# 0xPolygonZero/plonky2

Measured on AMD Instinct MI355X. Metric: LDE+Poseidon-commit GFE/s, higher is better.
Workload: dtype u64 (Goldilocks)

## Files before the change

### plonky2_amd/csrc/gl_mul3.hpp

```cpp
#pragma once
#include "asm_block.h"
#include "gl.hpp"

namespace gl {

#define P2_SA "v[70:71]", "v70", "v71", "v[72:73]", "v72", "v73", "v[74:75]", "v74", "v75", "s[40:41]", "s[42:43]"
#define P2_SB "v[76:77]", "v76", "v77", "v[78:79]", "v78", "v79", "v[80:81]", "v80", "v81", "s[44:45]", "s[46:47]"
#define P2_SC "v[82:83]", "v82", "v83", "v[84:85]", "v84", "v85", "v[86:87]", "v86", "v87", "s[48:49]", "s[50:51]"

#define P2_ST1(P, P0, P1, M, M0, M1, Q, Q0, Q1, C1, C2, a0, a1, b0, b1, r0, r1) "v_mad_u64_u32 " P ", " C1 ", %[" a0 "], %[" b0 "], 0\n\t"
#define P2_ST2(P, P0, P1, M, M0, M1, Q, Q0, Q1, C1, C2, a0, a1, b0, b1, r0, r1) "v_mad_u64_u32 " M ", " C1 ", %[" a1 "], %[" b0 "], 0\n\t"
#define P2_ST3(P, P0, P1, M, M0, M1, Q, Q0, Q1, C1, C2, a0, a1, b0, b1, r0, r1) "v_mad_u64_u32 " M ", " C2 ", %[" a0 "], %[" b1 "], " M "\n\t"
#define P2_ST4(P, P0, P1, M, M0, M1, Q, Q0, Q1, C1, C2, a0, a1, b0, b1, r0, r1) "v_mad_u64_u32 " Q ", " C1 ", %[" a1 "], %[" b1 "], 0\n\t"
#define P2_ST5(P, P0, P1, M, M0, M1, Q, Q0, Q1, C1, C2, a0, a1, b0, b1, r0, r1) "v_add_co_u32 " P1 ", " C1 ", " P1 ", " M0 "\n\t"
#define P2_ST6(P, P0, P1, M, M0, M1, Q, Q0, Q1, C1, C2, a0, a1, b0, b1, r0, r1) "v_addc_co_u32 " Q0 ", " C1 ", " Q0 ", " M1 ", " C1 "\n\t"
#define P2_ST7(P, P0, P1, M, M0, M1, Q, Q0, Q1, C1, C2, a0, a1, b0, b1, r0, r1) "v_addc_co_u32 " Q1 ", " C1 ", " Q1 ", 0, " C1 "\n\t"
#define P2_ST8(P, P0, P1, M, M0, M1, Q, Q0, Q1, C1, C2, a0, a1, b0, b1, r0, r1) "v_subb_co_u32 " P0 ", " C1 ", " P0 ", " Q1 ", " C2 "\n\t"
#define P2_ST9(P, P0, P1, M, M0, M1, Q, Q0, Q1, C1, C2, a0, a1, b0, b1, r0, r1) "v_subb_co_u32 " P1 ", " C1 ", " P1 ", 0, " C1 "\n\t"
#define P2_ST10(P, P0, P1, M, M0, M1, Q, Q0, Q1, C1, C2, a0, a1, b0, b1, r0, r1) "v_mad_u64_u32 " P ", " C2 ", " Q0 ", -1, " P "\n\t"
#define P2_ST11(P, P0, P1, M, M0, M1, Q, Q0, Q1, C1, C2, a0, a1, b0, b1, r0, r1) "v_cndmask_b32 " M0 ", 0, 1, " C2 "\n\t"
#define P2_ST12(P, P0, P1, M, M0, M1, Q, Q0, Q1, C1, C2, a0, a1, b0, b1, r0, r1) "v_subb_co_u32 " M0 ", " C1 ", " M0 ", 0, " C1 "\n\t"
#define P2_ST13(P, P0, P1, M, M0, M1, Q, Q0, Q1, C1, C2, a0, a1, b0, b1, r0, r1) "v_add_u32 " P1 ", " P1 ", " M0 "\n\t"
#define P2_ST14(P, P0, P1, M, M0, M1, Q, Q0, Q1, C1, C2, a0, a1, b0, b1, r0, r1) "v_mad_i64_i32 %[" r0 "], " C1 ", " M0 ", -1, " P "\n\t"

// ... 207 lines not shown
    return ra;
#endif
}

#define P2_FD1(P, P0, P1, M, M0, M1, Q, Q0, Q1, C1, C2, a0, a1, b0, b1, r0, r1) "v_mad_u64_u32 " P ", " C1 ", %[" b1 "], -1, %[" a0 "]\n\t"
#define P2_FD2(P, P0, P1, M, M0, M1, Q, Q0, Q1, C1, C2, a0, a1, b0, b1, r0, r1) "v_add_co_u32 " P1 ", " C1 ", " P1 ", %[" b0 "]\n\t"
#define P2_FD3(P, P0, P1, M, M0, M1, Q, Q0, Q1, C1, C2, a0, a1, b0, b1, r0, r1) "v_cndmask_b32 " M0 ", 0, -1, " C1 "\n\t"
#define P2_FD4(P, P0, P1, M, M0, M1, Q, Q0, Q1, C1, C2, a0, a1, b0, b1, r0, r1) "v_mad_u64_u32 %[" r0 "], " C1 ", " M0 ", 1, " P "\n\t"

__host__ __device__ __forceinline__ u64 fold_row_c(u64 al, u64 ah) {
    u32 k1;
    u32 w1 = addc32((u32)(al >> 32), (u32)ah, 0u, &k1);
    u32 w2 = (u32)(ah >> 32) + k1;
    u64 lo64 = ((u64)w1 << 32) | (u32)al;
    u64 t = (u64)w2 * 0xFFFFFFFFu + lo64;
    return fold_carry(t, t < lo64);
}

__device__ __forceinline__ void fold3(const u64 al[3], const u64 ah[3], u64 y[3]) {
    if (!P2_ASM_INTERPRETED()) {
        for (int k = 0; k < 3; ++k) y[k] = fold_row_c(al[k], ah[k]);
        return;
    }
    u64 ra, rb, rc;
    P2_ASM(P2_ROW(P2_FD1) P2_ROW(P2_FD2) P2_ROW(P2_FD3) P2_ROW(P2_FD4),
           (P2_O([ra0], "=&v", ra), P2_O([rb0], "=&v", rb), P2_O([rc0], "=&v", rc)),
           (P2_I([xa0], "v", al[0]), P2_I([ya0], "v", (u32)ah[0]), P2_I([ya1], "v", (u32)(ah[0] >> 32)),
            P2_I([xb0], "v", al[1]), P2_I([yb0], "v", (u32)ah[1]), P2_I([yb1], "v", (u32)(ah[1] >> 32)),
            P2_I([xc0], "v", al[2]), P2_I([yc0], "v", (u32)ah[2]), P2_I([yc1], "v", (u32)(ah[2] >> 32))),
           ("v70", "v71", "v72", "v76", "v77", "v78", "v82", "v83", "v84", "s40", "s41", "s44", "s45", "s48", "s49"));
    y[0] = ra;
    y[1] = rb;
    y[2] = rc;
}
__device__ __forceinline__ u64 fold1(u64 al, u64 ah) {
    if (!P2_ASM_INTERPRETED()) return fold_row_c(al, ah);
    u64 ra;
    P2_ASM(P2_A1(P2_FD1, P2_SA) P2_A1(P2_FD2, P2_SA) P2_NOP P2_A1(P2_FD3, P2_SA) P2_A1(P2_FD4, P2_SA),
           (P2_O([ra0], "=&v", ra)), (P2_I([xa0], "v", al), P2_I([ya0], "v", (u32)ah), P2_I([ya1], "v", (u32)(ah >> 32))),
           ("v70", "v71", "v72", "s40", "s41"));
    return ra;
}

#define P2_FW1(P, P0, P1, M, M0, M1, Q, Q0, Q1, C1, C2, a0, a1, b0, b1, r0, r1) "v_mad_u64_u32 " P ", " C1 ", %[" b1 "], -1, %[" a0 "]\n\t"
#define P2_FW2(P, P0, P1, M, M0, M1, Q, Q0, Q1, C1, C2, a0, a1, b0, b1, r0, r1) "v_cndmask_b32 " M0 ", 0, -1, " C1 "\n\t"
#define P2_FW3(P, P0, P1, M, M0, M1, Q, Q0, Q1, C1, C2, a0, a1, b0, b1, r0, r1) "v_mad_u64_u32 " P ", " C1 ", " M0 ", 1, " P "\n\t"
#define P2_FW4 P2_FD2
#define P2_FW5 P2_FD3
#define P2_FW6 P2_FD4

__host__ __device__ __forceinline__ u64 fold_row_wide_c(u64 al, u64 ah) {
    u64 t = (ah >> 32) * 0xFFFFFFFFull + al;
    t += t < al ? 0xFFFFFFFFull : 0;
    const u64 u = t + (ah << 32);
    return u + (u < t ? 0xFFFFFFFFull : 0);
}

__device__ __forceinline__ void fold3w(const u64 al[3], const u64 ah[3], u64 y[3]) {
    if (!P2_ASM_INTERPRETED()) {
        for (int k = 0; k < 3; ++k) y[k] = fold_row_wide_c(al[k], ah[k]);
        return;
    }
    u64 ra, rb, rc;
    P2_ASM(P2_ROW(P2_FW1) P2_ROW(P2_FW2) P2_ROW(P2_FW3) P2_ROW(P2_FW4) P2_ROW(P2_FW5) P2_ROW(P2_FW6),
           (P2_O([ra0], "=&v", ra), P2_O([rb0], "=&v", rb), P2_O([rc0], "=&v", rc)),
           (P2_I([xa0], "v", al[0]), P2_I([ya0], "v", (u32)ah[0]), P2_I([ya1], "v", (u32)(ah[0] >> 32)),
            P2_I([xb0], "v", al[1]), P2_I([yb0], "v", (u32)ah[1]), P2_I([yb1], "v", (u32)(ah[1] >> 32)),
            P2_I([xc0], "v", al[2]), P2_I([yc0], "v", (u32)ah[2]), P2_I([yc1], "v", (u32)(ah[2] >> 32))),
           ("v70", "v71", "v72", "v76", "v77", "v78", "v82", "v83", "v84", "s40", "s41", "s44", "s45", "s48", "s49"));
    y[0] = ra;
    y[1] = rb;
    y[2] = rc;
}
__device__ __forceinline__ u64 fold1w(u64 al, u64 ah) {
    if (!P2_ASM_INTERPRETED()) return fold_row_wide_c(al, ah);
    u64 ra;
    P2_ASM(P2_A1(P2_FW1, P2_SA) P2_NOP P2_A1(P2_FW2, P2_SA) P2_A1(P2_FW3, P2_SA) P2_A1(P2_FW4, P2_SA) P2_NOP P2_A1(P2_FW5, P2_SA)
               P2_A1(P2_FW6, P2_SA),
           (P2_O([ra0], "=&v", ra)), (P2_I([xa0], "v", al), P2_I([ya0], "v", (u32)ah), P2_I([ya1], "v", (u32)(ah >> 32))),
           ("v70", "v71", "v72", "s40", "s41"));
    return ra;
}

}
```

### plonky2_amd/csrc/merkle.hpp

```cpp
#pragma once
#include "poseidon.hpp"
#include "poseidon4.hpp"
#include "poseidon16.hpp"
#include "ntt.hpp"

namespace merkle {
using gl::u32;
using gl::u64;

struct ColMajorReader {
    const u64 *m;
    size_t stride;
    __device__ __forceinline__ u64 operator()(size_t L, unsigned e) const { return m[(size_t)e * stride + L]; }
};
struct RowMajorReader {
    const u64 *m;
    size_t W;
    __device__ __forceinline__ u64 operator()(size_t L, unsigned e) const { return m[L * W + e]; }
};
struct FriPlanarReader {
    const u64 *p0, *p1;
    unsigned arity_bits;
    __device__ __forceinline__ u64 operator()(size_t L, unsigned e) const {
        const u64 *p = (e & 1) ? p1 : p0;
        return p[(L << arity_bits) + (e >> 1)];
    }
};

struct DigestPrefixedReader {
    const u64 *prefix;
    const u64 *m;
    size_t stride;
    __device__ __forceinline__ u64 operator()(size_t L, unsigned e) const {
        return e < 4 ? prefix[4 * L + e] : m[(size_t)(e - 4) * stride + L];
    }
};

__device__ __forceinline__ u64 *node_slot(u64 *digests, u64 *cap, unsigned h, unsigned level, size_t j) {
    if (level == h) return cap + 4 * j;
    size_t s = j >> (h - level);
    size_t jl = j & (((size_t)1 << (h - level)) - 1);
    size_t sub_digests = 2 * (((size_t)1 << h) - 1);
    size_t idx = 2 * (((jl >> 1) << (level + 1)) + ((size_t)1 << level) - 1) + (jl & 1);
    return digests + 4 * (s * sub_digests + idx);
}

template <class Reader>
__global__ void __launch_bounds__(256) hash_leaves_kernel(Reader rd, unsigned W, size_t leaf_offset, size_t leaf_count,
                                                         unsigned h, u64 *digests, u64 *cap) {
    size_t t = (size_t)blockIdx.x * blockDim.x + threadIdx.x;
    if (t >= leaf_count) return;
    const size_t L = leaf_offset + t;
    u64 s[12];
#pragma unroll
    for (int i = 0; i < 12; ++i) s[i] = 0;
    if (W <= 4) {
        for (unsigned i = 0; i < W; ++i) s[i] = rd(L, i);
    } else {
        for (unsigned off = 0; off < W; off += 8) {
            unsigned cnt = W - off < 8 ? W - off : 8;
#pragma unroll
            for (unsigned i = 0; i < 8; ++i)
                if (i < cnt) s[i] = rd(L, off + i);
            const unsigned next = off + 8 < W ? (W - off - 8 < 8 ? W - off - 8 : 8) : 0;
            const unsigned keep = off + 8 < W ? (next == 8 ? 0x8u : (0xFu << (next / 3)) & 0xFu) : 0x1u;
            poseidon::permute(s, keep, off + 8 < W ? (next == 8 ? 8 : -1) : 3);
        }
    }
    u64 *dst = node_slot(digests, cap, h, 0, L);
#pragma unroll
    for (int i = 0; i < 4; ++i) dst[i] = gl::canon(s[i]);
}

template <class Reader>
__global__ void __launch_bounds__(256) hash_leaves_chunks_kernel(Reader rd, unsigned W, size_t leaf_offset, size_t leaf_count,
                                                                unsigned h, u64 *digests, u64 *cap, unsigned off_begin,
                                                                unsigned off_end, u64 *state, size_t state_stride) {
    size_t t = (size_t)blockIdx.x * blockDim.x + threadIdx.x;
    if (t >= leaf_count) return;
    const size_t L = leaf_offset + t;
    u64 s[12];
#pragma unroll
    for (int i = 0; i < 12; ++i) s[i] = 0;
    if (off_begin) {
        const unsigned nxt = W - off_begin < 8 ? W - off_begin : 8;
#pragma unroll
        for (unsigned i = 0; i < 12; ++i)
            if (i >= 3 * (nxt / 3)) s[i] = state[(size_t)i * state_stride + t];
    }
    for (unsigned off = off_begin; off < off_end; off += 8) {
        unsigned cnt = W - off < 8 ? W - off : 8;
#pragma unroll
        for (unsigned i = 0; i < 8; ++i)
            if (i < cnt) s[i] = rd(L, off + i);
        const unsigned next = off + 8 < W ? (W - off - 8 < 8 ? W - off - 8 : 8) : 0;
        const unsigned keep = off + 8 < W ? (next == 8 ? 0x8u : (0xFu << (next / 3)) & 0xFu) : 0x1u;
        poseidon::permute(s, keep, off + 8 < W ? (next == 8 ? 8 : -1) : 3);
    }
    if (off_end >= W) {
        u64 *dst = node_slot(digests, cap, h, 0, L);
#pragma unroll
        for (int i = 0; i < 4; ++i) dst[i] = gl::canon(s[i]);
    } else {
        const unsigned nxt = W - off_end < 8 ? W - off_end : 8;
#pragma unroll
        for (unsigned i = 0; i < 12; ++i)
            if (i >= 3 * (nxt / 3)) state[(size_t)i * state_stride + t] = s[i];
    }
}

__global__ void __launch_bounds__(256) merkle_level_kernel(u64 *digests, u64 *cap, unsigned h, unsigned level,
                                                          size_t n_nodes) {
    size_t j = (size_t)blockIdx.x * blockDim.x + threadIdx.x;
    if (j >= n_nodes) return;
    const u64 *ch = node_slot(digests, cap, h, level - 1, 2 * j);
    u64 out[4];
    poseidon::two_to_one(ch, ch + 4, out);
    u64 *dst = node_slot(digests, cap, h, level, j);
#pragma unroll
    for (int i = 0; i < 4; ++i) dst[i] = out[i];
}

template <class Reader>
__global__ void __launch_bounds__(256) hash_leaves_quad_kernel(Reader rd, unsigned W, size_t leaf_offset, size_t leaf_count,
                                                              unsigned h, u64 *digests, u64 *cap) {
    const size_t t = ((size_t)blockIdx.x * blockDim.x + threadIdx.x) >> 2;
    const unsigned q = threadIdx.x & 3;
    const bool live = t < leaf_count;
    const size_t L = leaf_offset + (live ? t : 0);
    u64 w[3] = {0, 0, 0};
    if (W <= 4) {
#pragma unroll
        for (unsigned u = 0; u < 3; ++u)
            if (live && 3 * q + u < W) w[u] = rd(L, 3 * q + u);
    } else {
        for (unsigned off = 0; off < W; off += 8) {
            const unsigned cnt = W - off < 8 ? W - off : 8;
#pragma unroll
            for (unsigned u = 0; u < 3; ++u) {
                const unsigned e = 3 * q + u;
                if (live && e < cnt) w[u] = rd(L, off + e);
            }
            poseidon4::permute_quad(w, q);
        }
    }
    if (live) {
        u64 *dst = node_slot(digests, cap, h, 0, L);
        if (q == 0) {
            dst[0] = gl::canon(w[0]);
            dst[1] = gl::canon(w[1]);
            dst[2] = gl::canon(w[2]);
        } else if (q == 1) {
            dst[3] = gl::canon(w[0]);
        }
    }
}

__global__ void __launch_bounds__(256) merkle_level_quad_kernel(u64 *digests, u64 *cap, unsigned h, unsigned level,
                                                               size_t n_nodes) {
    const size_t j = ((size_t)blockIdx.x * blockDim.x + threadIdx.x) >> 2;
    const unsigned q = threadIdx.x & 3;
    const bool live = j < n_nodes;
    const u64 *ch = node_slot(digests, cap, h, level - 1, 2 * (live ? j : 0));
    u64 w[3];
#pragma unroll
    for (unsigned u = 0; u < 3; ++u) w[u] = (live && 3 * q + u < 8) ? ch[3 * q + u] : 0;
    poseidon4::permute_quad(w, q);
    if (live) {
        u64 *dst = node_slot(digests, cap, h, level, j);
        if (q == 0) {
            dst[0] = gl::canon(w[0]);
            dst[1] = gl::canon(w[1]);
            dst[2] = gl::canon(w[2]);
        } else if (q == 1) {
            dst[3] = gl::canon(w[0]);
        }
    }
}

template <class Reader>
// ... 38 lines not shown
    if (live) states[12 * t + r] = gl::canon(w);
}

__global__ void permute_batch_kernel(u64 *states, size_t count) {
    size_t t = (size_t)blockIdx.x * blockDim.x + threadIdx.x;
    if (t >= count) return;
    u64 s[12];
#pragma unroll
    for (int i = 0; i < 12; ++i) s[i] = states[12 * t + i];
    poseidon::permute(s);
#pragma unroll
    for (int i = 0; i < 12; ++i) states[12 * t + i] = gl::canon(s[i]);
}

__global__ void field_selftest_kernel(const u64 *a, const u64 *b, size_t count, u64 *out) {
    size_t t = (size_t)blockIdx.x * blockDim.x + threadIdx.x;
    if (t >= count) return;
    const u64 x = a[t], y = b[t];
    out[t] = gl::canon(gl::mul(x, y));
    out[count + t] = gl::canon(gl::mul1(x, y));
    u64 aa[3] = {x, y, x}, bb[3] = {y, x, x}, rr[3];
    gl::mul3(aa, bb, rr);
    u64 ok = (gl::canon(rr[1]) == gl::canon(rr[0])) && (gl::canon(rr[2]) == gl::canon(gl::mul(x, x))) ? 0 : 1;
    if (gl::canon(gl::mul1_lowregs(x, y)) != gl::canon(gl::mul(x, y))) ok |= 2;
#define P2_CHK_POW2(S)                                                                                              \
    if (gl::canon(ntt::mul_pow2_asm<S>(x)) != gl::canon(gl::mul(x, (S) < 64 ? 1ull << ((S) & 63) : 0xFFFFFFFFull << (((S) - 64) & 31)))) \
        ok |= 4;
    P2_CHK_POW2(12) P2_CHK_POW2(24) P2_CHK_POW2(36) P2_CHK_POW2(48) P2_CHK_POW2(60) P2_CHK_POW2(72) P2_CHK_POW2(84)
    P2_CHK_POW2(1) P2_CHK_POW2(31) P2_CHK_POW2(33) P2_CHK_POW2(63) P2_CHK_POW2(65) P2_CHK_POW2(95)
#undef P2_CHK_POW2
    {
        const u64 al = x >> 1, ah = y >> 1;
        const u64 want = gl::canon(gl::add(al, gl::mul(ah, 1ull << 32)));
        if (gl::canon(gl::fold1(al, ah)) != want) ok |= 8;
        const u64 al3[3] = {al, ah, al ^ 0x2AAAAAAAAAAAAAAAull}, ah3[3] = {ah, al, ah};
        u64 y3[3];
        gl::fold3(al3, ah3, y3);
        for (int k = 0; k < 3; ++k)
            if (gl::canon(y3[k]) != gl::canon(gl::add(al3[k], gl::mul(ah3[k], 1ull << 32)))) ok |= 16;
    }
    {
        const u64 a2[2] = {x, y ^ 0x9E3779B97F4A7C15ull}, b2[2] = {y, x};
        u64 r2[2];
        gl::mul2(a2, b2, r2);
        if (gl::canon(r2[0]) != gl::canon(gl::mul(x, y)) || gl::canon(r2[1]) != gl::canon(gl::mul(a2[1], x))) ok |= 32;
    }
    if (gl::canon(gl::mul_add(x, y, x ^ y)) != gl::canon(gl::add(gl::mul(x, y), x ^ y)) || gl::canon(gl::mul_add(y, x, ~0ull)) != gl::canon(gl::add(gl::mul(x, y), ~0ull)) ||
        gl::canon(gl::mul_add(x, x, y)) != gl::canon(gl::add(gl::mul(x, x), y)))
        ok |= 128;
    {
        const u64 a3[3] = {x, y, x}, b3[3] = {y, x, x}, c3[3] = {x ^ y, ~0ull, y};
        u64 r3[3];
        gl::mad3(a3, b3, c3, r3);
        for (int k = 0; k < 3; ++k)
            if (gl::canon(r3[k]) != gl::canon(gl::add(gl::mul(a3[k], b3[k]), c3[k]))) ok |= 256;
    }
    {
        const u64 a3[3] = {x, y, x ^ 0x9E3779B97F4A7C15ull}, b3[3] = {y, y, x};
        u64 r3[3];
        gl::mul3cg(a3, b3, r3);
        for (int k = 0; k < 3; ++k)
            if (gl::canon(r3[k]) != gl::canon(gl::mul(a3[k], b3[k]))) ok |= 512;
        if (gl::canon(gl::mul1cg(x, y)) != gl::canon(gl::mul(x, y)) || gl::canon(gl::mul1cg(y, y)) != gl::canon(gl::mul(y, y))) ok |= 512;
    }
    {
        const u64 al3[3] = {x, y, x ^ y}, ah3[3] = {y, x, ~x};
        u64 y3[3];
        gl::fold3w(al3, ah3, y3);
        for (int k = 0; k < 3; ++k)
            if (gl::canon(y3[k]) != gl::canon(gl::add(al3[k], gl::mul(ah3[k], 1ull << 32)))) ok |= 1024;
        if (gl::canon(gl::fold1w(x, y)) != gl::canon(gl::add(x, gl::mul(y, 1ull << 32)))) ok |= 1024;
    }
    {
        const u64 z = x ^ 0x9E3779B97F4A7C15ull;
        const u64 a3[3][3] = {{x, y, z}, {y, z, x}, {z, x, y}}, b3[3][3] = {{y, y, x}, {y, x, y}, {x, y, y}};
        for (int j = 0; j < 3; ++j) {
            u64 r3[3];
            gl::mul3cx(a3[j], b3[j], r3);
            for (int k = 0; k < 3; ++k)
                if (gl::canon(r3[k]) != gl::canon(gl::mul(a3[j][k], b3[j][k]))) ok |= 2048;
        }
        if (gl::canon(gl::mul1cx(x, y)) != gl::canon(gl::mul(x, y)) || gl::canon(gl::mul1cx(y, y)) != gl::canon(gl::mul(y, y))) ok |= 2048;
    }
    out[2 * count + t] = gl::canon(rr[0]);
    out[5 * count + t] = ok;
    out[3 * count + t] = gl::canon(gl::add(x, y));
    out[4 * count + t] = gl::canon(gl::sub(x, y));
}

}
```

### plonky2_amd/csrc/poseidon.hpp

```cpp
#pragma once
#include "gl.hpp"
#include "gl_mul3.hpp"
#ifndef P2HOT_EMU
#define P2_CONST_QUAL __constant__
#endif
#define P2_LITERAL_QUAL static constexpr
#include "poseidon_constants.h"

namespace poseidon {
using gl::u32;
using gl::u64;

#define RC P2_POSEIDON_ALL_ROUND_CONSTANTS
#define RC_SPLIT P2_POSEIDON_PUSHED_ROUND_CONSTANTS_SPLIT

__device__ __forceinline__ u64 sbox7(u64 x) {
    u64 x2 = gl::sqr(x);
    u64 x4 = gl::sqr(x2);
    u64 x3 = gl::mul(x, x2);
    return gl::mul(x3, x4);
}

__device__ __forceinline__ u64 ark(u64 a, u64 c) {
    if (!P2_ASM_INTERPRETED()) return gl::add_canon(a, c);
// ... 46 lines not shown
    b = x[1];
    c = x[2];
}

__device__ __forceinline__ void sbox_layer(u64 s[12]) {
#pragma unroll
    for (int i = 0; i < 12; i += 3) sbox7_x3(s[i], s[i + 1], s[i + 2]);
}
__device__ __forceinline__ void sbox_layer_cx(u64 s[12]) {
#pragma unroll
    for (int i = 0; i < 12; i += 3) sbox7_x3cx(s[i], s[i + 1], s[i + 2]);
}

__device__ __forceinline__ u32 opaque_const(u32 c) {
#ifndef P2HOT_EMU
    asm volatile("" : "+s"(c));
#endif
    return c;
}

template <u32 C>
__device__ __forceinline__ void mds_term(u64 (&al)[3], u64 (&ah)[3], u32 l0, u32 h0, u32 l1, u32 h1, u32 l2, u32 h2) {
    if (!P2_ASM_INTERPRETED()) {
        al[0] += (u64)l0 * C;
        ah[0] += (u64)h0 * C;
        al[1] += (u64)l1 * C;
        ah[1] += (u64)h1 * C;
        al[2] += (u64)l2 * C;
        ah[2] += (u64)h2 * C;
        return;
    }
    u64 d;
    P2_ASM_NC("v_mad_u64_u32 %0, %6, %7, %13, %0\n\t"
              "v_mad_u64_u32 %1, %6, %8, %13, %1\n\t"
              "v_mad_u64_u32 %2, %6, %9, %13, %2\n\t"
              "v_mad_u64_u32 %3, %6, %10, %13, %3\n\t"
              "v_mad_u64_u32 %4, %6, %11, %13, %4\n\t"
              "v_mad_u64_u32 %5, %6, %12, %13, %5",
              (P2_O(, "+v", al[0]), P2_O(, "+v", ah[0]), P2_O(, "+v", al[1]), P2_O(, "+v", ah[1]), P2_O(, "+v", al[2]),
               P2_O(, "+v", ah[2]), P2_O(, "=&s", d)),
              (P2_I(, "v", l0), P2_I(, "v", h0), P2_I(, "v", l1), P2_I(, "v", h1), P2_I(, "v", l2), P2_I(, "v", h2),
               P2_I(, "n", C)));
}
template <bool HAS_K>
__device__ __forceinline__ void mds_first(u64 (&al)[3], u64 (&ah)[3], u32 l0, u32 h0, u32 l1, u32 h1, u32 l2, u32 h2,
                                          const u64 *k) {
    if (!P2_ASM_INTERPRETED()) {
        const u64 z[6] = {0, 0, 0, 0, 0, 0};
        const u64 *kk = HAS_K ? k : z;
        al[0] = (u64)l0 * 17u + kk[0];
        ah[0] = (u64)h0 * 17u + kk[1];
        al[1] = (u64)l1 * 17u + kk[2];
        ah[1] = (u64)h1 * 17u + kk[3];
        al[2] = (u64)l2 * 17u + kk[4];
        ah[2] = (u64)h2 * 17u + kk[5];
        return;
    }
    u64 d;
    if (HAS_K) {
        P2_ASM_NC("v_mad_u64_u32 %0, %6, %7, 17, %13\n\t"
                  "v_mad_u64_u32 %1, %6, %8, 17, %14\n\t"
                  "v_mad_u64_u32 %2, %6, %9, 17, %15\n\t"
                  "v_mad_u64_u32 %3, %6, %10, 17, %16\n\t"
                  "v_mad_u64_u32 %4, %6, %11, 17, %17\n\t"
                  "v_mad_u64_u32 %5, %6, %12, 17, %18",
                  (P2_O(, "=&v", al[0]), P2_O(, "=&v", ah[0]), P2_O(, "=&v", al[1]), P2_O(, "=&v", ah[1]),
                   P2_O(, "=&v", al[2]), P2_O(, "=&v", ah[2]), P2_O(, "=&s", d)),
                  (P2_I(, "v", l0), P2_I(, "v", h0), P2_I(, "v", l1), P2_I(, "v", h1), P2_I(, "v", l2), P2_I(, "v", h2),
                   P2_I(, "s", k[0]), P2_I(, "s", k[1]), P2_I(, "s", k[2]), P2_I(, "s", k[3]), P2_I(, "s", k[4]),
                   P2_I(, "s", k[5])));
    } else {
        P2_ASM_NC("v_mad_u64_u32 %0, %6, %7, 17, 0\n\t"
                  "v_mad_u64_u32 %1, %6, %8, 17, 0\n\t"
                  "v_mad_u64_u32 %2, %6, %9, 17, 0\n\t"
                  "v_mad_u64_u32 %3, %6, %10, 17, 0\n\t"
                  "v_mad_u64_u32 %4, %6, %11, 17, 0\n\t"
                  "v_mad_u64_u32 %5, %6, %12, 17, 0",
                  (P2_O(, "=&v", al[0]), P2_O(, "=&v", ah[0]), P2_O(, "=&v", al[1]), P2_O(, "=&v", ah[1]),
                   P2_O(, "=&v", al[2]), P2_O(, "=&v", ah[2]), P2_O(, "=&s", d)),
                  (P2_I(, "v", l0), P2_I(, "v", h0), P2_I(, "v", l1), P2_I(, "v", h1), P2_I(, "v", l2), P2_I(, "v", h2)));
    }
}

template <int R>
__device__ __forceinline__ u64 mds_row(const u32 (&xl)[12], const u32 (&xh)[12]) {
    static_assert(R > 0 && R < 12, "row 0 carries the diagonal term");
    constexpr u32 C[12] = {17, 15, 41, 16, 2, 28, 13, 13, 39, 18, 34, 20};
    u64 al = (u64)xl[R] * opaque_const(C[0]), ah = (u64)xh[R] * opaque_const(C[0]);
#pragma unroll
    for (int i = 1; i < 12; ++i) {
        al += (u64)xl[(R + i) % 12] * opaque_const(C[i]);
        ah += (u64)xh[(R + i) % 12] * opaque_const(C[i]);
    }
    return gl::fold1(al, ah);
}

__device__ __forceinline__ void mds_layer(u64 s[12], const u64 *rc2, unsigned groups = 0xFu, int single = -1) {
    u32 xl[12], xh[12];
#pragma unroll
    for (int i = 0; i < 12; ++i) {
        xl[i] = (u32)s[i];
        xh[i] = (u32)(s[i] >> 32);
    }
#pragma unroll
    for (int g = 0; g < 12; g += 3) {
        if (!(groups >> (g / 3) & 1u)) continue;
        u64 al[3], ah[3], y[3];
#define P2_X(i) xl[(g + (i)) % 12], xh[(g + (i)) % 12], xl[(g + (i) + 1) % 12], xh[(g + (i) + 1) % 12], xl[(g + (i) + 2) % 12], xh[(g + (i) + 2) % 12]
        if (rc2)
            mds_first<true>(al, ah, P2_X(0), rc2 + 2 * g);
        else
            mds_first<false>(al, ah, P2_X(0), nullptr);
        mds_term<15>(al, ah, P2_X(1));
        mds_term<41>(al, ah, P2_X(2));
        mds_term<16>(al, ah, P2_X(3));
        mds_term<2>(al, ah, P2_X(4));
        mds_term<28>(al, ah, P2_X(5));
        mds_term<13>(al, ah, P2_X(6));
        mds_term<13>(al, ah, P2_X(7));
        mds_term<39>(al, ah, P2_X(8));
        mds_term<18>(al, ah, P2_X(9));
        mds_term<34>(al, ah, P2_X(10));
        mds_term<20>(al, ah, P2_X(11));
#undef P2_X
        if (g == 0) {
            al[0] += (u64)xl[0] * opaque_const(8);
            ah[0] += (u64)xh[0] * opaque_const(8);
        }
        gl::fold3(al, ah, y);
        s[g] = y[0];
        s[g + 1] = y[1];
        s[g + 2] = y[2];
    }
    if (single == 3)
        s[3] = mds_row<3>(xl, xh);
    else if (single == 8)
        s[8] = mds_row<8>(xl, xh);
}

struct Mat12 {
    u32 v[144];
};
constexpr Mat12 mds_matrix() {
    Mat12 m{};
    for (int r = 0; r < 12; ++r)
        for (int c = 0; c < 12; ++c) m.v[12 * r + c] = P2_POSEIDON_M1_ROW0[(c - r + 12) % 12] - ((c - r + 12) % 12 == 0 ? 8u : 0u) + (r == 0 && c == 0 ? 8u : 0u);
    return m;
}
constexpr Mat12 mat_mul(const Mat12 &a, const Mat12 &b) {
    Mat12 m{};
    for (int r = 0; r < 12; ++r)
        for (int c = 0; c < 12; ++c) {
            u64 acc = 0;
            for (int k = 0; k < 12; ++k) acc += (u64)a.v[12 * r + k] * b.v[12 * k + c];
            m.v[12 * r + c] = (u32)acc;
        }
    return m;
}
constexpr bool mat_checks() {
    const Mat12 m1 = mds_matrix(), m2 = mat_mul(m1, m1), m3 = mat_mul(m1, m2);
    for (int j = 0; j < 12; ++j) {
        if (m1.v[j] != P2_POSEIDON_M1_ROW0[j] || m2.v[j] != P2_POSEIDON_M2_ROW0[j]) return false;
        if (m1.v[12 * j] != P2_POSEIDON_MCOL0[j] || m2.v[12 * j] != P2_POSEIDON_MCOL0[12 + j]) return false;
    }
    for (int i = 0; i < 144; ++i)
        if (m3.v[i] != P2_POSEIDON_M3[i]) return false;
    return true;
}
static_assert(mat_checks(), "M, M^2, M^3: the compile-time products disagree with the generated tables");
constexpr Mat12 mat_drop_col0(const Mat12 &a) {
    Mat12 m = a;
    for (int r = 0; r < 12; ++r) m.v[12 * r] = 0;
    return m;
}
P2_LITERAL_QUAL Mat12 MDS1 = mds_matrix();
P2_LITERAL_QUAL Mat12 MDM = mat_mul(mat_drop_col0(mds_matrix()), mds_matrix());
P2_LITERAL_QUAL Mat12 MDMDM = mat_mul(mat_drop_col0(mds_matrix()), mat_mul(mat_drop_col0(mds_matrix()), mds_matrix()));
P2_LITERAL_QUAL Mat12 MDMDMDM = mat_mul(mat_drop_col0(mds_matrix()), MDMDM);

constexpr bool pass4_rows_fit() {
    const Mat12 m1 = mds_matrix(), md = mat_drop_col0(m1);
    const Mat12 p1 = mat_mul(md, m1), p2 = mat_mul(md, p1), p3 = mat_mul(md, p2);
    for (int i = 0; i < 144; ++i)
        if (p1.v[i] != MDM.v[i] || p2.v[i] != MDMDM.v[i] || p3.v[i] != MDMDMDM.v[i]) return false;
    for (int r = 0; r < 12; ++r) {
        u64 sum = (u64)p2.v[12 * r] + p1.v[12 * r] + m1.v[12 * r];
        for (int c = 0; c < 12; ++c) {
            u64 e = 0;
            for (int k = 0; k < 12; ++k) e += (u64)md.v[12 * r + k] * p2.v[12 * k + c];
            if (e != p3.v[12 * r + c]) return false;
            sum += e;
        }
        if (sum > (1ull << 32)) return false;
    }
    return true;
}
static_assert(pass4_rows_fit(), "(MD)^3 M: a four-application row would overflow its 64-bit chains");

template <bool FIRST = false>
__device__ __forceinline__ void partial_rounds4(u64 s[12], u64 c1, u64 c2, u64 c3, u64 cn) {
    u32 xl[12], xh[12];
    const u64 z0 = FIRST ? s[0] : sbox7_cx(s[0]);
    xl[0] = (u32)z0;
    xh[0] = (u32)(z0 >> 32);
#pragma unroll
    for (int i = 1; i < 12; ++i) {
        xl[i] = (u32)s[i];
        xh[i] = (u32)(s[i] >> 32);
    }
    u64 al = (u32)c1, ah = c1 >> 32;
#pragma unroll
    for (int j = 0; j < 12; ++j) {
        al += (u64)xl[j] * P2_POSEIDON_M1_ROW0[j];
        ah += (u64)xh[j] * P2_POSEIDON_M1_ROW0[j];
    }
    const u64 s1 = sbox7_cx(gl::fold1(al, ah));
    const u32 s1l = (u32)s1, s1h = (u32)(s1 >> 32);
    al = (u64)s1l * MDS1.v[0] + (u32)c2;
    ah = (u64)s1h * MDS1.v[0] + (c2 >> 32);
#pragma unroll
    for (int j = 0; j < 12; ++j) {
        al += (u64)xl[j] * MDM.v[j];
        ah += (u64)xh[j] * MDM.v[j];
    }
    const u64 s2 = sbox7_cx(gl::fold1(al, ah));
    const u32 s2l = (u32)s2, s2h = (u32)(s2 >> 32);
    al = (u64)s1l * MDM.v[0] + (u64)s2l * MDS1.v[0] + (u32)c3;
    ah = (u64)s1h * MDM.v[0] + (u64)s2h * MDS1.v[0] + (c3 >> 32);
#pragma unroll
    for (int j = 0; j < 12; ++j) {
        al += (u64)xl[j] * MDMDM.v[j];
        ah += (u64)xh[j] * MDMDM.v[j];
    }
    const u64 s3 = sbox7_cx(gl::fold1(al, ah));
    const u32 s3l = (u32)s3, s3h = (u32)(s3 >> 32);
#pragma unroll
    for (int g = 0; g < 12; g += 3) {
        u64 bl[3], bh[3], y[3];
#pragma unroll
        for (int t = 0; t < 3; ++t) {
            const int i = g + t;
            bl[t] = (u64)s1l * MDMDM.v[12 * i] + (u64)s2l * MDM.v[12 * i] + (u64)s3l * MDS1.v[12 * i] + (i == 0 ? (u64)(u32)cn : 0);
            bh[t] = (u64)s1h * MDMDM.v[12 * i] + (u64)s2h * MDM.v[12 * i] + (u64)s3h * MDS1.v[12 * i] + (i == 0 ? cn >> 32 : 0);
#pragma unroll
            for (int j = 0; j < 12; ++j) {
                bl[t] += (u64)xl[j] * MDMDMDM.v[12 * i + j];
                bh[t] += (u64)xh[j] * MDMDMDM.v[12 * i + j];
            }
        }
        gl::fold3w(bl, bh, y);
        s[g] = y[0];
        s[g + 1] = y[1];
        s[g + 2] = y[2];
    }
}

__device__ __forceinline__ void partial_rounds3(u64 s[12], u64 c1, u64 c2, const u64 *cv) {
    u32 xl[12], xh[12];
    const u64 z0 = sbox7_cx(s[0]);
    xl[0] = (u32)z0;
    xh[0] = (u32)(z0 >> 32);
#pragma unroll
    for (int i = 1; i < 12; ++i) {
        xl[i] = (u32)s[i];
        xh[i] = (u32)(s[i] >> 32);
    }
    u64 al = (u32)c1, ah = c1 >> 32;
#pragma unroll
    for (int j = 0; j < 12; ++j) {
        al += (u64)xl[j] * P2_POSEIDON_M1_ROW0[j];
        ah += (u64)xh[j] * P2_POSEIDON_M1_ROW0[j];
    }
    const u64 s1 = sbox7_cx(gl::fold1(al, ah));
    const u32 s1l = (u32)s1, s1h = (u32)(s1 >> 32);
    al = (u64)s1l * MDS1.v[0] + (u32)c2;
    ah = (u64)s1h * MDS1.v[0] + (c2 >> 32);
#pragma unroll
    for (int j = 0; j < 12; ++j) {
        al += (u64)xl[j] * MDM.v[j];
        ah += (u64)xh[j] * MDM.v[j];
    }
    const u64 s2 = sbox7_cx(gl::fold1(al, ah));
    const u32 s2l = (u32)s2, s2h = (u32)(s2 >> 32);
#pragma unroll
    for (int g = 0; g < 12; g += 3) {
        u64 bl[3], bh[3], y[3];
#pragma unroll
        for (int t = 0; t < 3; ++t) {
            const int i = g + t;
            const u64 ci = cv[i];
            bl[t] = (u64)s1l * MDM.v[12 * i] + (u64)s2l * MDS1.v[12 * i] + (u32)ci;
            bh[t] = (u64)s1h * MDM.v[12 * i] + (u64)s2h * MDS1.v[12 * i] + (ci >> 32);
#pragma unroll
            for (int j = 0; j < 12; ++j) {
                bl[t] += (u64)xl[j] * MDMDM.v[12 * i + j];
                bh[t] += (u64)xh[j] * MDMDM.v[12 * i + j];
            }
        }
        gl::fold3(bl, bh, y);
        s[g] = y[0];
        s[g + 1] = y[1];
        s[g + 2] = y[2];
    }
}

__device__ inline void permute(u64 s[12], unsigned out_groups = 0xFu, int out_single = -1) {
    const u32 z0 = opaque_zero();
#pragma unroll
    for (int i = 0; i < 12; ++i) s[i] = ark(s[i], RC[i + z0]);
    int round = 0;
#pragma unroll 1
    for (int k = 0; k < 3; ++k, ++round) {
        sbox_layer_cx(s);
        mds_layer(s, RC_SPLIT + 24 * (round + 1));
    }
    sbox_layer_cx(s);
    partial_rounds4<true>(s, P2_POSEIDON_PUSHED_ROUND_CONSTANTS[12 * 4], P2_POSEIDON_PUSHED_ROUND_CONSTANTS[12 * 5],
                          P2_POSEIDON_PUSHED_ROUND_CONSTANTS[12 * 6], P2_POSEIDON_PUSHED_ROUND_CONSTANTS[12 * 7]);
    round = 7;
#pragma unroll 1
    for (int k = 0; k < 4; ++k, round += 4)
        partial_rounds4(s, P2_POSEIDON_PUSHED_ROUND_CONSTANTS[12 * (round + 1)], P2_POSEIDON_PUSHED_ROUND_CONSTANTS[12 * (round + 2)],
                        P2_POSEIDON_PUSHED_ROUND_CONSTANTS[12 * (round + 3)], P2_POSEIDON_PUSHED_ROUND_CONSTANTS[12 * (round + 4)]);
    const u32 z26 = opaque_zero();
    partial_rounds3(s, P2_POSEIDON_PUSHED_ROUND_CONSTANTS[12 * 24], P2_POSEIDON_PUSHED_ROUND_CONSTANTS[12 * 25],
                    P2_POSEIDON_PUSHED_ROUND_CONSTANTS + 12 * 26 + z26);
    round = 26;
#pragma unroll 1
    for (int k = 0; k < 3; ++k, ++round) {
        sbox_layer_cx(s);
        mds_layer(s, RC_SPLIT + 24 * (round + 1));
    }
    sbox_layer_cx(s);
    mds_layer(s, nullptr, out_groups, out_single);
}

__device__ __forceinline__ void two_to_one(const u64 l[4], const u64 r[4], u64 out[4]) {
    u64 s[12];
#pragma unroll
    for (int i = 0; i < 4; ++i) {
        s[i] = l[i];
        s[4 + i] = r[i];
        s[8 + i] = 0;
    }
    permute(s, 0x1u, 3);
#pragma unroll
    for (int i = 0; i < 4; ++i) out[i] = gl::canon(s[i]);
}

#undef RC
#undef RC_SPLIT
}
```

Before: 22.21.

## Use exec-masked inline-asm folds with pinned register homes in Poseidon leaf hashing

Adds new inline-asm Goldilocks fold and add-round-constant helpers that reduce via a single mad plus an exec-masked correction, with outputs pinned to fixed VGPR homes per state group. The Poseidon permutation is templated on a MASKED flag and uses these helpers for leaf hashing with column-major, row-major and FRI readers. Those kernels also gain a launch-bounds minimum of 4 blocks per CU to raise occupancy. The aim is fewer ALU instructions per modular reduction and less register movement. In exchange it relies on hard-coded register assignments and exec manipulation, which could cause spills or miscompiles, and it adds self-tests.

Result: no change. 22.34 (median of 6 runs) (+0.6%).

```diff
diff --git a/plonky2_amd/csrc/gl_mul3.hpp b/plonky2_amd/csrc/gl_mul3.hpp
--- a/plonky2_amd/csrc/gl_mul3.hpp
+++ b/plonky2_amd/csrc/gl_mul3.hpp
@@ -313,4 +313,117 @@
     return ra;
 }
 
-}
+#define P2_FX1(H, HH, C, a0, b0, b1) "v_mad_u64_u32 " H ", " C ", %[" b1 "], -1, %[" a0 "]\n\t"
+#define P2_FX2(H, HH, C, a0, b0, b1) "v_add_co_u32 " HH ", " C ", " HH ", %[" b0 "]\n\t"
+#define P2_FXM(H, HH, C, a0, b0, b1) "s_and_b64 exec, " C ", s[52:53]\n\tv_mad_u64_u32 " H ", s[42:43], 1, -1, " H "\n\t"
+#define P2_AX1(H, HH, C, a0, b0, b1) "v_mad_u64_u32 " H ", " C ", %[" b0 "], 1, %[" a0 "]\n\t"
+#define P2_AX2(H, HH, C, a0, b0, b1) "v_add_co_u32 " HH ", " C ", " HH ", %[" b1 "]\n\t"
+#define P2_FXROW(ST, PA, HA, PB, HB, PC, HC) \
+    ST(PA, HA, "s[40:41]", "xa0", "ya0", "ya1") ST(PB, HB, "s[44:45]", "xb0", "yb0", "yb1") ST(PC, HC, "s[48:49]", "xc0", "yc0", "yc1")
+#define P2_FX_NARROW3(...) P2_CX_SAVE P2_FXROW(P2_FX1, __VA_ARGS__) P2_FXROW(P2_FX2, __VA_ARGS__) P2_FXROW(P2_FXM, __VA_ARGS__) P2_CX_REST
+#define P2_FX_WIDE3(...)                                                                                                          \
+    P2_CX_SAVE P2_FXROW(P2_FX1, __VA_ARGS__) P2_FXROW(P2_FXM, __VA_ARGS__) P2_CX_REST P2_FXROW(P2_FX2, __VA_ARGS__)               \
+        P2_FXROW(P2_FXM, __VA_ARGS__) P2_CX_REST
+#define P2_AX_3(...) P2_CX_SAVE P2_FXROW(P2_AX1, __VA_ARGS__) P2_FXROW(P2_AX2, __VA_ARGS__) P2_FXROW(P2_FXM, __VA_ARGS__) P2_CX_REST
+#define P2_FX_CLOBBERS3 "s40", "s41", "s42", "s43", "s44", "s45", "s48", "s49", "s52", "s53", "scc"
+#define P2_FX_CLOBBERS1 "s40", "s41", "s42", "s43", "s52", "s53", "scc"
+
+template <int G>
+__device__ __forceinline__ void fold3x(const u64 al[3], const u64 ah[3], u64 y[3]);
+template <int G>
+__device__ __forceinline__ void fold3wx(const u64 al[3], const u64 ah[3], u64 y[3]);
+template <int G>
+__device__ __forceinline__ void ark3x(const u64 a[3], const u64 c[3], u64 y[3]);
+template <int K>
+__device__ __forceinline__ u64 fold1x(u64 al, u64 ah);
+template <int K>
+__device__ __forceinline__ u64 fold1wx(u64 al, u64 ah);
+
+#ifdef P2HOT_EMU
+template <int G>
+__device__ __forceinline__ void fold3x(const u64 al[3], const u64 ah[3], u64 y[3]) {
+    for (int k = 0; k < 3; ++k) y[k] = fold_row_c(al[k], ah[k]);
+}
+template <int G>
+__device__ __forceinline__ void fold3wx(const u64 al[3], const u64 ah[3], u64 y[3]) {
+    for (int k = 0; k < 3; ++k) y[k] = fold_row_wide_c(al[k], ah[k]);
+}
+template <int G>
+__device__ __forceinline__ void ark3x(const u64 a[3], const u64 c[3], u64 y[3]) {
+    for (int k = 0; k < 3; ++k) y[k] = add_canon(a[k], c[k]);
+}
+template <int K>
+__device__ __forceinline__ u64 fold1x(u64 al, u64 ah) {
+    return fold_row_c(al, ah);
+}
+template <int K>
+__device__ __forceinline__ u64 fold1wx(u64 al, u64 ah) {
+    return fold_row_wide_c(al, ah);
+}
+#else
+#define P2_ASM_X(...) P2_ASM(__VA_ARGS__)
+#define P2_FX_IO3(PA, PB, PC, XCON, X0, X1, X2, Y0, Y1, Y2)                                                                        \
+    (P2_O([ra0], "=&{" PA "}", ra), P2_O([rb0], "=&{" PB "}", rb), P2_O([rc0], "=&{" PC "}", rc)),                                 \
+        (P2_I([xa0], XCON, X0), P2_I([ya0], "v", (u32)(Y0)), P2_I([ya1], "v", (u32)((Y0) >> 32)), P2_I([xb0], XCON, X1),             \
+         P2_I([yb0], "v", (u32)(Y1)), P2_I([yb1], "v", (u32)((Y1) >> 32)), P2_I([xc0], XCON, X2), P2_I([yc0], "v", (u32)(Y2)),       \
+         P2_I([yc1], "v", (u32)((Y2) >> 32))),                                                                                     \
+        (P2_FX_CLOBBERS3)
+#define P2_DEF_FOLD3X(G, PA, HA, PB, HB, PC, HC)                                                                   \
+    template <>                                                                                                    \
+    __device__ __forceinline__ void fold3x<G>(const u64 al[3], const u64 ah[3], u64 y[3]) {                        \
+        u64 ra, rb, rc;                                                                                            \
+        P2_ASM_X(P2_FX_NARROW3(PA, HA, PB, HB, PC, HC), P2_FX_IO3(PA, PB, PC, "v", al[0], al[1], al[2], ah[0], ah[1], ah[2])); \
+        y[0] = ra, y[1] = rb, y[2] = rc;                                                                           \
+    }                                                                                                              \
+    template <>                                                                                                    \
+    __device__ __forceinline__ void fold3wx<G>(const u64 al[3], const u64 ah[3], u64 y[3]) {                       \
+        u64 ra, rb, rc;                                                                                            \
+        P2_ASM_X(P2_FX_WIDE3(PA, HA, PB, HB, PC, HC), P2_FX_IO3(PA, PB, PC, "v", al[0], al[1], al[2], ah[0], ah[1], ah[2])); \
+        y[0] = ra, y[1] = rb, y[2] = rc;                                                                           \
+    }                                                                                                              \
+    template <>                                                                                                    \
+    __device__ __forceinline__ void ark3x<G>(const u64 a[3], const u64 c[3], u64 y[3]) {                           \
+        u64 ra, rb, rc;                                                                                            \
+        P2_ASM_X(P2_AX_3(PA, HA, PB, HB, PC, HC), P2_FX_IO3(PA, PB, PC, "s", c[0], c[1], c[2], a[0], a[1], a[2]));   \
+        y[0] = ra, y[1] = rb, y[2] = rc;                                                                           \
+    }
+#define P2_FX_IO1(PA)                                                                                                              \
+    (P2_O([ra0], "=&{" PA "}", ra)), (P2_I([xa0], "v", al), P2_I([ya0], "v", (u32)ah), P2_I([ya1], "v", (u32)(ah >> 32))), (P2_FX_CLOBBERS1)
+#define P2_FXA(ST, PA, HA) ST(PA, HA, "s[40:41]", "xa0", "ya0", "ya1")
+#define P2_DEF_FOLD1X(K, PA, HA)                                                                                                     \
+    template <>                                                                                                                      \
+    __device__ __forceinline__ u64 fold1x<K>(u64 al, u64 ah) {                                                                       \
+        u64 ra;                                                                                                                      \
+        P2_ASM_X(P2_CX_SAVE P2_FXA(P2_FX1, PA, HA) P2_FXA(P2_FX2, PA, HA) P2_FXA(P2_FXM, PA, HA) P2_CX_REST, P2_FX_IO1(PA));           \
+        return ra;                                                                                                                   \
+    }                                                                                                                                \
+    template <>                                                                                                                      \
+    __device__ __forceinline__ u64 fold1wx<K>(u64 al, u64 ah) {                                                                      \
+        u64 ra;                                                                                                                      \
+        P2_ASM_X(P2_CX_SAVE P2_FXA(P2_FX1, PA, HA) P2_FXA(P2_FXM, PA, HA) P2_CX_REST P2_FXA(P2_FX2, PA, HA) P2_FXA(P2_FXM, PA, HA)     \
+                   P2_CX_REST,                                                                                                       \
+               P2_FX_IO1(PA));                                                                                                       \
+        return ra;                                                                                                                   \
+    }
+P2_DEF_FOLD3X(0, "v[94:95]", "v95", "v[96:97]", "v97", "v[98:99]", "v99")
+P2_DEF_FOLD3X(3, "v[100:101]", "v101", "v[102:103]", "v103", "v[104:105]", "v105")
+P2_DEF_FOLD3X(6, "v[106:107]", "v107", "v[108:109]", "v109", "v[110:111]", "v111")
+P2_DEF_FOLD3X(9, "v[112:113]", "v113", "v[114:115]", "v115", "v[116:117]", "v117")
+P2_DEF_FOLD3X(12, "v[70:71]", "v71", "v[76:77]", "v77", "v[82:83]", "v83")
+P2_DEF_FOLD1X(12, "v[118:119]", "v119")
+#endif
+
+#define P2_FX_AT(NAME)                                                                              \
+    __device__ __forceinline__ void NAME##_at(int g, const u64 a[3], const u64 b[3], u64 y[3]) {    \
+        switch (g) {                                                                                \
+            case 0: NAME<0>(a, b, y); break;                                                        \
+            case 3: NAME<3>(a, b, y); break;                                                        \
+            case 6: NAME<6>(a, b, y); break;                                                        \
+            default: NAME<9>(a, b, y); break;                                                       \
+        }                                                                                           \
+    }
+P2_FX_AT(fold3x)
+P2_FX_AT(fold3wx)
+#undef P2_FX_AT
+
+}
diff --git a/plonky2_amd/csrc/merkle.hpp b/plonky2_amd/csrc/merkle.hpp
--- a/plonky2_amd/csrc/merkle.hpp
+++ b/plonky2_amd/csrc/merkle.hpp
@@ -9,16 +9,19 @@
 using gl::u64;
 
 struct ColMajorReader {
+    static constexpr bool masked_folds = true;
     const u64 *m;
     size_t stride;
     __device__ __forceinline__ u64 operator()(size_t L, unsigned e) const { return m[(size_t)e * stride + L]; }
 };
 struct RowMajorReader {
+    static constexpr bool masked_folds = true;
     const u64 *m;
     size_t W;
     __device__ __forceinline__ u64 operator()(size_t L, unsigned e) const { return m[L * W + e]; }
 };
 struct FriPlanarReader {
+    static constexpr bool masked_folds = true;
     const u64 *p0, *p1;
     unsigned arity_bits;
     __device__ __forceinline__ u64 operator()(size_t L, unsigned e) const {
@@ -28,6 +31,7 @@
 };
 
 struct DigestPrefixedReader {
+    static constexpr bool masked_folds = false;
     const u64 *prefix;
     const u64 *m;
     size_t stride;
@@ -46,7 +50,7 @@
 }
 
 template <class Reader>
-__global__ void __launch_bounds__(256) hash_leaves_kernel(Reader rd, unsigned W, size_t leaf_offset, size_t leaf_count,
+__global__ void __launch_bounds__(256, Reader::masked_folds ? 4 : 1) hash_leaves_kernel(Reader rd, unsigned W, size_t leaf_offset, size_t leaf_count,
                                                          unsigned h, u64 *digests, u64 *cap) {
     size_t t = (size_t)blockIdx.x * blockDim.x + threadIdx.x;
     if (t >= leaf_count) return;
@@ -64,7 +68,7 @@
                 if (i < cnt) s[i] = rd(L, off + i);
             const unsigned next = off + 8 < W ? (W - off - 8 < 8 ? W - off - 8 : 8) : 0;
             const unsigned keep = off + 8 < W ? (next == 8 ? 0x8u : (0xFu << (next / 3)) & 0xFu) : 0x1u;
-            poseidon::permute(s, keep, off + 8 < W ? (next == 8 ? 8 : -1) : 3);
+            poseidon::permute<Reader::masked_folds>(s, keep, off + 8 < W ? (next == 8 ? 8 : -1) : 3);
         }
     }
     u64 *dst = node_slot(digests, cap, h, 0, L);
@@ -95,7 +99,7 @@
             if (i < cnt) s[i] = rd(L, off + i);
         const unsigned next = off + 8 < W ? (W - off - 8 < 8 ? W - off - 8 : 8) : 0;
         const unsigned keep = off + 8 < W ? (next == 8 ? 0x8u : (0xFu << (next / 3)) & 0xFu) : 0x1u;
-        poseidon::permute(s, keep, off + 8 < W ? (next == 8 ? 8 : -1) : 3);
+        poseidon::permute<false>(s, keep, off + 8 < W ? (next == 8 ? 8 : -1) : 3);
     }
     if (off_end >= W) {
         u64 *dst = node_slot(digests, cap, h, 0, L);
@@ -300,6 +304,48 @@
         }
         if (gl::canon(gl::mul1cx(x, y)) != gl::canon(gl::mul(x, y)) || gl::canon(gl::mul1cx(y, y)) != gl::canon(gl::mul(y, y))) ok |= 2048;
     }
+#define P2_CHK_X3(FN, G, A3, B3, WANT, BIT)                                            \
+    _Pragma("unroll") for (int j = 0; j < 3; ++j) {                                                      \
+        const u64 ar[3] = {A3[j], A3[(j + 1) % 3], A3[(j + 2) % 3]};                   \
+        const u64 br[3] = {B3[j], B3[(j + 1) % 3], B3[(j + 2) % 3]};                   \
+        u64 yr[3];                                                                     \
+        gl::FN<G>(ar, br, yr);                                                         \
+        for (int k = 0; k < 3; ++k)                                                    \
+            if (gl::canon(yr[k]) != WANT(ar[k], br[k])) ok |= BIT;                     \
+    }
+#define P2_CHK_X3_HOMES(FN, A3, B3, WANT, BIT) \
+    P2_CHK_X3(FN, 0, A3, B3, WANT, BIT) P2_CHK_X3(FN, 3, A3, B3, WANT, BIT) P2_CHK_X3(FN, 6, A3, B3, WANT, BIT) P2_CHK_X3(FN, 9, A3, B3, WANT, BIT) \
+        P2_CHK_X3(FN, 12, A3, B3, WANT, BIT)
+#define P2_WANT_FOLD(AL, AH) gl::canon(gl::add(AL, gl::mul(AH, 1ull << 32)))
+#define P2_WANT_ADD(A, C) gl::canon(gl::add(A, C))
+    {
+        const u64 al = x >> 1, ah = y >> 1;
+        const u64 al3[3] = {al, ah, al ^ 0x2AAAAAAAAAAAAAAAull}, ah3[3] = {ah, al, ah ^ 0x7FFFFFFF00000000ull};
+        P2_CHK_X3_HOMES(fold3x, al3, ah3, P2_WANT_FOLD, 4096)
+        if (gl::canon(gl::fold1x<12>(al, ah)) != P2_WANT_FOLD(al, ah) || gl::canon(gl::fold1x<12>(ah, al)) != P2_WANT_FOLD(ah, al) ||
+            gl::canon(gl::fold1x<12>(al3[2], ah3[2])) != P2_WANT_FOLD(al3[2], ah3[2]))
+            ok |= 4096;
+    }
+    {
+        const u64 al3[3] = {x, y, x ^ y}, ah3[3] = {y, x, ~x};
+        P2_CHK_X3_HOMES(fold3wx, al3, ah3, P2_WANT_FOLD, 8192)
+        if (gl::canon(gl::fold1wx<12>(x, y)) != P2_WANT_FOLD(x, y) || gl::canon(gl::fold1wx<12>(y, x)) != P2_WANT_FOLD(y, x) ||
+            gl::canon(gl::fold1wx<12>(~x, ~y)) != P2_WANT_FOLD(~x, ~y))
+            ok |= 8192;
+    }
+    {
+        const u64 cs[6] = {0, 1, 0xFFFFFFFFull, 1ull << 32, gl::P - (1ull << 32), gl::P - 1};
+        const u64 a3[3] = {x, y, ~x};
+#pragma unroll
+        for (int i = 0; i < 6; i += 3) {
+            const u64 c3[3] = {cs[i], cs[i + 1], cs[i + 2]};
+            P2_CHK_X3_HOMES(ark3x, a3, c3, P2_WANT_ADD, 16384)
+        }
+    }
+#undef P2_CHK_X3
+#undef P2_CHK_X3_HOMES
+#undef P2_WANT_FOLD
+#undef P2_WANT_ADD
     out[2 * count + t] = gl::canon(rr[0]);
     out[5 * count + t] = ok;
     out[3 * count + t] = gl::canon(gl::add(x, y));
diff --git a/plonky2_amd/csrc/poseidon.hpp b/plonky2_amd/csrc/poseidon.hpp
--- a/plonky2_amd/csrc/poseidon.hpp
+++ b/plonky2_amd/csrc/poseidon.hpp
@@ -152,7 +152,7 @@
     }
 }
 
-template <int R>
+template <int R, bool MASKED = true>
 __device__ __forceinline__ u64 mds_row(const u32 (&xl)[12], const u32 (&xh)[12]) {
     static_assert(R > 0 && R < 12, "row 0 carries the diagonal term");
     constexpr u32 C[12] = {17, 15, 41, 16, 2, 28, 13, 13, 39, 18, 34, 20};
@@ -162,9 +162,11 @@
         al += (u64)xl[(R + i) % 12] * opaque_const(C[i]);
         ah += (u64)xh[(R + i) % 12] * opaque_const(C[i]);
     }
-    return gl::fold1(al, ah);
-}
-
+    return MASKED ? gl::fold1x<12>(al, ah) : gl::fold1(al, ah);
+}
+
+enum { MDS_PLAIN = 0, MDS_HOME = 1, MDS_LAST = 2 };
+template <int FOLD = MDS_PLAIN>
 __device__ __forceinline__ void mds_layer(u64 s[12], const u64 *rc2, unsigned groups = 0xFu, int single = -1) {
     u32 xl[12], xh[12];
 #pragma unroll
@@ -197,15 +199,20 @@
             al[0] += (u64)xl[0] * opaque_const(8);
             ah[0] += (u64)xh[0] * opaque_const(8);
         }
-        gl::fold3(al, ah, y);
+        if (FOLD == MDS_PLAIN)
+            gl::fold3(al, ah, y);
+        else if (FOLD == MDS_LAST)
+            gl::fold3x<12>(al, ah, y);
+        else
+            gl::fold3x_at(g, al, ah, y);
         s[g] = y[0];
         s[g + 1] = y[1];
         s[g + 2] = y[2];
     }
     if (single == 3)
-        s[3] = mds_row<3>(xl, xh);
+        s[3] = mds_row<3, FOLD != MDS_PLAIN>(xl, xh);
     else if (single == 8)
-        s[8] = mds_row<8>(xl, xh);
+        s[8] = mds_row<8, FOLD != MDS_PLAIN>(xl, xh);
 }
 
 struct Mat12 {
@@ -267,7 +274,7 @@
 }
 static_assert(pass4_rows_fit(), "(MD)^3 M: a four-application row would overflow its 64-bit chains");
 
-template <bool FIRST = false>
+template <bool FIRST = false, bool MASKED = true>
 __device__ __forceinline__ void partial_rounds4(u64 s[12], u64 c1, u64 c2, u64 c3, u64 cn) {
     u32 xl[12], xh[12];
     const u64 z0 = FIRST ? s[0] : sbox7_cx(s[0]);
@@ -284,7 +291,7 @@
         al += (u64)xl[j] * P2_POSEIDON_M1_ROW0[j];
         ah += (u64)xh[j] * P2_POSEIDON_M1_ROW0[j];
     }
-    const u64 s1 = sbox7_cx(gl::fold1(al, ah));
+    const u64 s1 = sbox7_cx(MASKED ? gl::fold1x<12>(al, ah) : gl::fold1(al, ah));
     const u32 s1l = (u32)s1, s1h = (u32)(s1 >> 32);
     al = (u64)s1l * MDS1.v[0] + (u32)c2;
     ah = (u64)s1h * MDS1.v[0] + (c2 >> 32);
@@ -293,7 +300,7 @@
         al += (u64)xl[j] * MDM.v[j];
         ah += (u64)xh[j] * MDM.v[j];
     }
-    const u64 s2 = sbox7_cx(gl::fold1(al, ah));
+    const u64 s2 = sbox7_cx(MASKED ? gl::fold1x<12>(al, ah) : gl::fold1(al, ah));
     const u32 s2l = (u32)s2, s2h = (u32)(s2 >> 32);
     al = (u64)s1l * MDM.v[0] + (u64)s2l * MDS1.v[0] + (u32)c3;
     ah = (u64)s1h * MDM.v[0] + (u64)s2h * MDS1.v[0] + (c3 >> 32);
@@ -302,7 +309,7 @@
         al += (u64)xl[j] * MDMDM.v[j];
         ah += (u64)xh[j] * MDMDM.v[j];
     }
-    const u64 s3 = sbox7_cx(gl::fold1(al, ah));
+    const u64 s3 = sbox7_cx(MASKED ? gl::fold1x<12>(al, ah) : gl::fold1(al, ah));
     const u32 s3l = (u32)s3, s3h = (u32)(s3 >> 32);
 #pragma unroll
     for (int g = 0; g < 12; g += 3) {
@@ -318,13 +325,17 @@
                 bh[t] += (u64)xh[j] * MDMDMDM.v[12 * i + j];
             }
         }
-        gl::fold3w(bl, bh, y);
+        if (MASKED)
+            gl::fold3wx<12>(bl, bh, y);
+        else
+            gl::fold3w(bl, bh, y);
         s[g] = y[0];
         s[g + 1] = y[1];
         s[g + 2] = y[2];
     }
 }
 
+template <bool MASKED = true>
 __device__ __forceinline__ void partial_rounds3(u64 s[12], u64 c1, u64 c2, const u64 *cv) {
     u32 xl[12], xh[12];
     const u64 z0 = sbox7_cx(s[0]);
@@ -341,7 +352,7 @@
         al += (u64)xl[j] * P2_POSEIDON_M1_ROW0[j];
         ah += (u64)xh[j] * P2_POSEIDON_M1_ROW0[j];
     }
-    const u64 s1 = sbox7_cx(gl::fold1(al, ah));
+    const u64 s1 = sbox7_cx(MASKED ? gl::fold1x<12>(al, ah) : gl::fold1(al, ah));
     const u32 s1l = (u32)s1, s1h = (u32)(s1 >> 32);
     al = (u64)s1l * MDS1.v[0] + (u32)c2;
     ah = (u64)s1h * MDS1.v[0] + (c2 >> 32);
@@ -350,7 +361,7 @@
         al += (u64)xl[j] * MDM.v[j];
         ah += (u64)xh[j] * MDM.v[j];
     }
-    const u64 s2 = sbox7_cx(gl::fold1(al, ah));
+    const u64 s2 = sbox7_cx(MASKED ? gl::fold1x<12>(al, ah) : gl::fold1(al, ah));
     const u32 s2l = (u32)s2, s2h = (u32)(s2 >> 32);
 #pragma unroll
     for (int g = 0; g < 12; g += 3) {
@@ -367,42 +378,57 @@
                 bh[t] += (u64)xh[j] * MDMDM.v[12 * i + j];
             }
         }
-        gl::fold3(bl, bh, y);
+        if (MASKED)
+            gl::fold3x_at(g, bl, bh, y);
+        else
+            gl::fold3(bl, bh, y);
         s[g] = y[0];
         s[g + 1] = y[1];
         s[g + 2] = y[2];
     }
 }
 
+template <bool MASKED = true>
 __device__ inline void permute(u64 s[12], unsigned out_groups = 0xFu, int out_single = -1) {
     const u32 z0 = opaque_zero();
-#pragma unroll
-    for (int i = 0; i < 12; ++i) s[i] = ark(s[i], RC[i + z0]);
+    if (!MASKED) {
+#pragma unroll
+        for (int i = 0; i < 12; ++i) s[i] = ark(s[i], RC[i + z0]);
+    }
+#pragma unroll
+    for (int g = 0; g < 12 && MASKED; g += 3) {
+        const u64 c[3] = {RC[g + z0], RC[g + 1 + z0], RC[g + 2 + z0]};
+        u64 y[3];
+        gl::ark3x<12>(s + g, c, y);
+        s[g] = y[0];
+        s[g + 1] = y[1];
+        s[g + 2] = y[2];
+    }
     int round = 0;
 #pragma unroll 1
     for (int k = 0; k < 3; ++k, ++round) {
         sbox_layer_cx(s);
-        mds_layer(s, RC_SPLIT + 24 * (round + 1));
+        mds_layer<MASKED ? MDS_HOME : MDS_PLAIN>(s, RC_SPLIT + 24 * (round + 1));
     }
     sbox_layer_cx(s);
-    partial_rounds4<true>(s, P2_POSEIDON_PUSHED_ROUND_CONSTANTS[12 * 4], P2_POSEIDON_PUSHED_ROUND_CONSTANTS[12 * 5],
+    partial_rounds4<true, MASKED>(s, P2_POSEIDON_PUSHED_ROUND_CONSTANTS[12 * 4], P2_POSEIDON_PUSHED_ROUND_CONSTANTS[12 * 5],
                           P2_POSEIDON_PUSHED_ROUND_CONSTANTS[12 * 6], P2_POSEIDON_PUSHED_ROUND_CONSTANTS[12 * 7]);
     round = 7;
 #pragma unroll 1
     for (int k = 0; k < 4; ++k, round += 4)
-        partial_rounds4(s, P2_POSEIDON_PUSHED_ROUND_CONSTANTS[12 * (round + 1)], P2_POSEIDON_PUSHED_ROUND_CONSTANTS[12 * (round + 2)],
+        partial_rounds4<false, MASKED>(s, P2_POSEIDON_PUSHED_ROUND_CONSTANTS[12 * (round + 1)], P2_POSEIDON_PUSHED_ROUND_CONSTANTS[12 * (round + 2)],
                         P2_POSEIDON_PUSHED_ROUND_CONSTANTS[12 * (round + 3)], P2_POSEIDON_PUSHED_ROUND_CONSTANTS[12 * (round + 4)]);
     const u32 z26 = opaque_zero();
-    partial_rounds3(s, P2_POSEIDON_PUSHED_ROUND_CONSTANTS[12 * 24], P2_POSEIDON_PUSHED_ROUND_CONSTANTS[12 * 25],
+    partial_rounds3<MASKED>(s, P2_POSEIDON_PUSHED_ROUND_CONSTANTS[12 * 24], P2_POSEIDON_PUSHED_ROUND_CONSTANTS[12 * 25],
                     P2_POSEIDON_PUSHED_ROUND_CONSTANTS + 12 * 26 + z26);
     round = 26;
 #pragma unroll 1
     for (int k = 0; k < 3; ++k, ++round) {
         sbox_layer_cx(s);
-        mds_layer(s, RC_SPLIT + 24 * (round + 1));
+        mds_layer<MASKED ? MDS_HOME : MDS_PLAIN>(s, RC_SPLIT + 24 * (round + 1));
     }
     sbox_layer_cx(s);
-    mds_layer(s, nullptr, out_groups, out_single);
+    mds_layer<MASKED ? MDS_LAST : MDS_PLAIN>(s, nullptr, out_groups, out_single);
 }
 
 __device__ __forceinline__ void two_to_one(const u64 l[4], const u64 r[4], u64 out[4]) {
```
